# Lcressot/fhe-string-bounty

Measured on AMD Instinct MI355X. Metric: PBS/sec (whole node), higher is better.
Workload: dtype f64

## Files before the change

fhe-string-bounty_amd/csrc/engine.h:

```cpp
#pragma once
#include <hip/hip_runtime.h>
#include <stdint.h>

#include <algorithm>
#include <map>
#include <memory>
#include <mutex>
#include <string>
#include <vector>

#include "../../include/fhestr.h"
#include "blind_rotate.h"
#include "device_buffer.h"
#include "engine_settings.h"
#include "grid_spans.h"

#define FHESTR_KERNEL_REVISION "r04.2"

namespace fhe {

inline uint32_t n_ggsw(const fhe_params_t& p) {
    return p.grouping_factor > 1 ? p.n / p.grouping_factor * (1u << p.grouping_factor) : p.n;
}
inline uint64_t multi_bit_key_bit(const uint64_t* group_bits, uint32_t g, uint32_t sel) {
    uint64_t prod = 1;
    for (uint32_t b = 0; b < g; b++) prod *= group_bits[b] ^ (((sel >> (g - 1 - b)) & 1) ^ 1);
    return prod;
}

void aes128_round_keys(const uint8_t key[16], uint8_t rk[11][16]);
const uint8_t* aes_sbox();

extern thread_local std::string g_last_error;
inline int under(const char* who, hipError_t e) { return e == hipSuccess ? 0 : fail(std::string(who) + ": " + hipGetErrorString(e)); }
inline int under(const char* who, int rc) { return rc ? fail(std::string(who) + ": " + g_last_error) : 0; }

uint64_t fill_accumulator(const fhe_params_t& p, const uint64_t* table, std::vector<uint64_t>& acc);
void fill_accumulator_torus(const fhe_params_t& p, const uint64_t* box_values, std::vector<uint64_t>& acc);

struct ByteRange { const char* lo; const char* hi; };
inline bool overlap(const ByteRange& a, const ByteRange& b) { return a.lo < b.hi && b.lo < a.hi; }

struct PipeLane {
    hipStream_t stream = nullptr;
    hipEvent_t done = nullptr;
    DeviceBuffer<uint64_t> small;
    DeviceBuffer<int8_t> digits;
    std::vector<ByteRange> ins, outs;
    bool blocks(const ByteRange& in, const ByteRange& out) const {
        for (const auto& w : outs)
            if (overlap(in, w) || overlap(out, w)) return true;
        for (const auto& r : ins)
            if (overlap(out, r)) return true;
        return false;
    }
    void remember(const ByteRange& in, const ByteRange& out) { add(ins, in); add(outs, out); }
    static void add(std::vector<ByteRange>& rs, const ByteRange& a) {
        for (auto& r : rs)
            if (r.lo == a.lo && r.hi == a.hi) return;
        if (rs.size() < 32) { rs.push_back(a); return; }
        rs[0].lo = std::min(rs[0].lo, a.lo);
        rs[0].hi = std::max(rs[0].hi, a.hi);
    }
};

struct Pipeline {
    static constexpr int MAX_LANES = 4;
    PipeLane lane[MAX_LANES];
    int ready = 0;
    int width = 2;
    uint64_t calls = 0;
    hipEvent_t input_ready = nullptr;
    hipEvent_t ks_done[2] = {nullptr, nullptr}, rot_done[2] = {nullptr, nullptr};
    ByteRange prev_out[2] = {{nullptr, nullptr}, {nullptr, nullptr}};
    hipEvent_t run_start = nullptr;

    template <class F> void each_event(F f) {
        for (auto& l : lane) f(l.done);
        for (int s = 0; s < 2; s++) { f(ks_done[s]); f(rot_done[s]); }
        f(run_start);
    }
    int ensure(int n);
    hipStream_t stream_of(int q, hipStream_t engine) const { return q ? lane[q].stream : engine; }
    int wait_others();
    int wait_all(hipStream_t engine);
    void end_run();
    void destroy(int keep = 0);
    ~Pipeline() { destroy(); }
};
static_assert(EngineSettings::OVERLAP_MAX == Pipeline::MAX_LANES, "every width the settings accept has its lane");

struct Engine;
struct Packing {
    Engine* e = nullptr;
    DeviceBuffer<int8_t> key;
    fhe_packing_params_t pp{0, 0};
    DeviceBuffer<int8_t> digits;
    DeviceBuffer<uint64_t> pack_in, pack_out;
    uint32_t pack_last[5] = {0, 0, 0, 0, 0};
    DeviceBuffer<uint64_t> unpack_in, unpack_out;
    uint32_t unpack_last[4] = {0, 0, 0, 0};
    DeviceBuffer<uint64_t> narrow_in, narrow_out;
    uint32_t narrow_last[5] = {0, 0, 0, 0, 0};
    void pack_info(uint32_t out[5]) const { std::copy(pack_last, pack_last + 5, out); }
    void unpack_info(uint32_t out[4]) const { std::copy(unpack_last, unpack_last + 4, out); }
    void narrow_info(uint32_t out[5]) const { std::copy(narrow_last, narrow_last + 5, out); }

    int load_key(const fhe_packing_params_t& pp, const uint64_t* pksk);
    int pack_dev(const uint64_t* d_cts, uint32_t count, uint64_t* d_glwes);
    int pack_host(const uint64_t* cts, uint32_t count, uint64_t* glwes);
    int extract_dev(const char* who, uint32_t k, uint32_t N, const uint64_t* d_glwes, uint32_t first, uint32_t count, uint64_t* d_cts, uint32_t* chunks = nullptr);
    int unpack_dev(const uint64_t* d_glwes, uint32_t first, uint32_t count, int refresh, uint64_t* d_cts);
    int unpack_host(const uint64_t* glwes, uint32_t first, uint32_t count, int refresh, uint64_t* cts);
    int narrow_dev(const uint64_t* d_glwes, uint32_t held, uint32_t bits, uint64_t* d_narrow);
    int narrow_host(const uint64_t* glwes, uint32_t held, uint32_t bits, uint64_t* narrow);
    int widen_dev(const uint64_t* d_narrow, uint32_t held, uint32_t bits, uint64_t* d_glwes);
    int widen_shape_dev(const char* who, uint32_t k, uint32_t N, const uint64_t* d_narrow, uint32_t held, uint32_t bits, uint64_t* d_glwes);
    int unpack_narrow_dev(const uint64_t* d_narrow, uint32_t held, uint32_t bits, uint32_t first, uint32_t count, int refresh, uint64_t* d_cts);
    int unpack_narrow_host(const uint64_t* narrow, uint32_t held, uint32_t bits, uint32_t first, uint32_t count, int refresh, uint64_t* cts);

    DeviceBuffer<uint32_t> ring_key;
    fhe_packing_params_t ring_pp{0, 0};
    DeviceBuffer<uint32_t> ring_tw;
    uint32_t ring_n_inv = 0;
    DeviceBuffer<uint64_t> ring_slots;
    DeviceBuffer<unsigned char> ring_tmp;
    uint64_t ring_last[5] = {0, 0, 0, 0, 0};
    int load_ring_key(const fhe_packing_params_t& pp, const uint64_t* key);
    int ring_pack_dev(const uint64_t* d_cts, uint32_t count, uint64_t* d_glwes);
    int ring_pack_host(const uint64_t* cts, uint32_t count, uint64_t* glwes);
    int ring_ntt_host(uint32_t N, int inverse, uint32_t* polys, uint32_t count);
};

struct Transcipher {
    Engine* e = nullptr;
    uint32_t cipher = 0, max_streams = 0, bits = 0;
    uint32_t n_streams = 0;
    int32_t round = 0;
    DeviceBuffer<uint64_t> key;
    DeviceBuffer<uint64_t> ring;
    DeviceBuffer<uint64_t> pbs_in;
    DeviceBuffer<uint32_t> tables;
    DeviceBuffer<uint8_t> ivs, data;
    DeviceBuffer<uint64_t> out;
    uint32_t lut_of[20] = {};
    uint32_t warm_rounds = 0, data_rounds = 0;
    uint64_t pbs_rows = 0;
    bool timed = false;
    double phase_ms[3] = {0, 0, 0};
    uint32_t timed_rounds = 0;
    hipEvent_t ev[4] = {nullptr, nullptr, nullptr, nullptr};

    static int create(Engine& e, uint32_t cipher, const uint64_t* key_cts, uint32_t max_streams, Transcipher** out);
    ~Transcipher();
    int begin(const uint8_t* ivs_host, uint32_t streams);
    int next(const uint8_t* data_host, uint32_t n_bytes, int refresh, uint64_t* out_host, uint64_t* d_out);
    int run_round(uint32_t rows, uint32_t n_bytes, uint32_t m, uint64_t* d_blocks);
    void info(uint32_t out[8]) const;
};

struct CastKey {
    Engine* e = nullptr;
    fhe_cast_params_t cp{};
    int32_t shift = 0;
    uint32_t in_dim = 0, out_size = 0;
    DeviceBuffer<int8_t> key;
    DeviceBuffer<int8_t> digits;
    DeviceBuffer<uint64_t> rows;
    DeviceBuffer<uint64_t> bodies;
    DeviceBuffer<uint64_t> lwes;
    DeviceBuffer<uint64_t> glwes;
    DeviceBuffer<uint32_t> idx;
    DeviceBuffer<unsigned char> meta;
    DeviceBuffer<uint64_t> in, out;
    bool fused = true;
    uint32_t group = 1;
    uint32_t meta_count = 0;
    uint32_t lut = 0;
    bool lut_ready = false;
    uint32_t last = 0;
    double v_in = 1.0;

    static int create(Engine& e, const fhe_cast_params_t& cp, const uint64_t* key, CastKey** out);
    int set_group(uint32_t group);
    int gate(const char* who) const;
    int keyswitch_dev(const uint64_t* d_src, uint32_t first, uint32_t count, bool packed, uint64_t* d_rows);
    int cast_dev(const uint64_t* d_src, uint32_t first, uint32_t count, bool packed, int mode, uint64_t* d_out);
    int cast_host(const uint64_t* src, uint32_t first, uint32_t count, bool packed, int mode, uint64_t* out);
    int cast_narrow_dev(const uint64_t* d_narrow, uint32_t held, uint32_t bits, uint32_t first, uint32_t count, int mode, uint64_t* d_out);
    int cast_narrow_host(const uint64_t* narrow, uint32_t held, uint32_t bits, uint32_t first, uint32_t count, int mode, uint64_t* out);
    int digits_host(const uint64_t* src, uint32_t first, uint32_t count, bool packed, int8_t* out, size_t* bytes);
    void info(uint32_t out[8]) const;
};

struct Engine {
    std::recursive_mutex mu;
    fhe_params_t p{};
    int device = 0;
    hipStream_t stream = nullptr;
    hipStream_t own_stream = nullptr;
    std::map<std::vector<uint64_t>, uint32_t> lut_dedup;
    std::vector<hipEvent_t> ring;
    size_t ring_used = 0;
    const BrVariant* variant = nullptr;
    const BrVariant* variant_large = nullptr;
    int cu_count = 256;
    uint32_t max_grid[3] = {0x7FFFFFFFu, 65535u, 65535u};
    GridSpans spans(uint64_t count, int axis) const { return grid_spans(count, max_grid[axis]); }
    int one_span(const char* who, uint64_t count, int axis) const {
        if (spans(count, axis).spans == 1) return 0;
        return fail(std::string(who) + ": grid." + "xyz"[axis] + " = " + std::to_string(count) + " does not fit one launch (the device allows " +
                    std::to_string(max_grid[axis]) + ")");
    }
    EngineSettings cfg;
    int pipeline = 0;
    Pipeline pipe;
    int sync_all_streams() { return pipe.wait_all(stream); }
    int leave_pipelined_run() {
        if (!pipeline) return 0;
        if (sync_all_streams()) return 1;
        pipe.end_run();
        return 0;
    }
    template <class T>
    int reserve_idle(DeviceBuffer<T>& b, size_t need) {
        if (b.bytes >= need) return 0;
        if (b.ptr && sync_all_streams()) return 1;
        return b.reserve(need);
    }
    int shadow_fit = -1;

    DeviceBuffer<uint32_t> d_ksk_packed;
    DeviceBuffer<uint64_t> d_ksk_rowsum;
    DeviceBuffer<int8_t> d_ksk_mfma;
    DeviceBuffer<double> d_fbsk;
    DeviceBuffer<double> d_fbsk_dense;
    DeviceBuffer<uint64_t> d_luts;
    uint32_t n_luts = 0;

    DeviceBuffer<uint64_t> d_in, d_out, d_pool;
    DeviceBuffer<uint32_t> d_idx;
    DeviceBuffer<unsigned char> d_meta;
    DeviceBuffer<uint64_t> d_compact;
    DeviceBuffer<unsigned char> d_ws;
    DeviceBuffer<uint32_t> d_slot_exp;
    MultiCuRuntime multi_cu;
    uint32_t ks_last[5] = {0, 0, 0, 0, 0};
    Packing packing;
    DeviceBuffer<uint32_t> refresh_idx;
    std::vector<std::unique_ptr<Transcipher>> transciphers;
    std::vector<std::unique_ptr<CastKey>> cast_keys;

    static int create(const fhe_params_t& p, int device, Engine** out);
    ~Engine();
    int use();
    int set_variant(int logR);
    int allow_rotate_lds();
    int load_keys(const uint64_t* bsk_std, const uint64_t* ksk);
    int load_seeded_keys(const uint8_t ksk_seed[16], const uint64_t* ksk_bodies, const uint8_t bsk_seed[16], const uint64_t* bsk_bodies,
                         uint64_t* bsk_std_out, uint64_t* ksk_out);
    int expand_seeded_lwe(const uint8_t* seeds, const uint64_t* bodies, uint32_t count, uint64_t* d_out, uint64_t* host_out);
    int expand_compact_list(const uint64_t* list, uint32_t count, uint64_t* d_out, uint64_t* host_out);
    int expand_compact_list_dev(const uint64_t* d_list, uint32_t count, uint64_t* d_out);
    int generate_keys(const uint64_t* glwe_sk, const uint64_t* small_sk, const uint8_t seed[32],
                      uint64_t* bsk_std_out, uint64_t* ksk_out);
    int install_keys(DeviceBuffer<uint64_t>&& d_ksk_std, DeviceBuffer<uint64_t>&& d_bsk_std);
    int convert_polys(const uint64_t* d_std, double* d_out, uint32_t n_polys);
    int convert_dense_key(const uint64_t* d_std, uint32_t n_polys);
    int probe_slot_exponents();
    uint64_t fill_accumulator(const uint64_t* table, std::vector<uint64_t>& acc) const { return fhe::fill_accumulator(p, table, acc); }
    int lut_upload_dedup(const std::vector<uint64_t>& acc, uint32_t* id);
    int set_stream(hipStream_t s, bool use_own);
    int lut_upload(const uint64_t* acc, uint32_t* id);
    int lut_download(uint32_t id, uint64_t* acc);
    int ensure_batch(uint32_t count);
    int timing_events(hipEvent_t*& e4);
    int check_lut_idx(const uint32_t* lut_idx, uint32_t count) const;

    int launch_keyswitch(const uint64_t* d_big, uint64_t* d_sm, uint32_t count, DeviceBuffer<int8_t>& digits, hipStream_t on = nullptr, bool shadow = false);
    int launch_blind_rotate(const uint64_t* d_sm, const uint32_t* d_lut_idx, uint64_t* d_big, uint32_t count, hipStream_t on = nullptr, bool two_per_cu = false,
                            bool one_workgroup_only = false);
    bool shadow_keyswitch_fits();
    int refresh_rows_dev(uint64_t* d_cts, uint32_t count);
    uint32_t rotate_registers() const;
    void keyswitch_info(uint32_t info[6]) const;
    int ks_pbs_dev(const uint64_t* d_big_in, const uint32_t* d_lut_idx, uint64_t* d_big_out, uint32_t count, bool allow_pipeline = false);
    int ks_pbs_host(const uint64_t* in, const uint32_t* lut_idx, uint64_t* out, uint32_t count);
    int keyswitch_host(const uint64_t* in, uint64_t* out_small, uint32_t count);
    int pbs_host(const uint64_t* in_small, const uint32_t* lut_idx, uint64_t* out, uint32_t count);
    int pbs_ks_host(const uint64_t* in_small, const uint32_t* lut_idx, uint64_t* out_small, uint32_t count);
    int lincomb_dev(const uint64_t* d_pool, const uint32_t* d_off, const uint32_t* d_src,
                    const int32_t* d_coeff, const uint64_t* d_cst, uint64_t* d_out, uint32_t jobs);
    int lincomb_rows_dev(const uint64_t* d_pool, const uint32_t* d_off, const uint32_t* d_src, const int32_t* d_coeff, const uint64_t* d_cst,
                         uint64_t* d_out, uint32_t jobs, uint32_t row_words);
    int lincomb_batch_dev(const uint64_t* d_pool, const uint32_t* d_off, const uint32_t* d_src, const int32_t* d_coeff,
                          const uint64_t* d_cst, uint64_t* d_out, uint32_t jobs, uint32_t instances, uint32_t src_slot, uint32_t src_inst,
                          uint32_t out_job, uint32_t out_inst, const uint32_t* d_lut_in, uint32_t* d_lut_out);
    int restride_dev(const uint64_t* d_in, uint64_t* d_out, uint32_t slots, uint32_t instances, uint32_t in_slot, uint32_t in_inst,
                     uint32_t out_slot, uint32_t out_inst);
    int lincomb_host(const uint64_t* pool, uint32_t pool_count, const uint32_t* off, const uint32_t* src,
                     const int32_t* coeff, const uint64_t* cst, uint64_t* out, uint32_t jobs);
    int transcipher_init_host(uint32_t cipher, uint32_t S, const uint64_t* key, const uint8_t* ivs, uint64_t* ring);
    int transcipher_gather_host(uint32_t cipher, uint32_t S, int32_t round, uint32_t rows, const uint64_t* ring, const uint64_t* key, const uint8_t* ivs,
                                const uint8_t* data, uint32_t n_bytes, uint32_t m, uint64_t* pbs_in, uint32_t* tables);
    int transcipher_apply_host(uint32_t cipher, uint32_t S, int32_t round, const uint64_t* ring, uint32_t n_bytes, uint32_t m, uint64_t* out);
    int last_kernel_ms(float ms[2]);
    int kernel_times(double total_ms[2], uint32_t* calls, bool reset);
    int synchronize();
};

struct Seed256;
size_t compact_dim(const fhe_params_t& p);
int compact_pk_generate(const fhe_params_t& p, const uint64_t* big_sk, const Seed256& seed, uint64_t* pk, int threads);

int params_supported(const fhe_params_t& p);
int packing_params_check(const fhe_params_t& p, const fhe_packing_params_t& pp);
void packing_unpack_noise(const fhe_params_t& p, const fhe_packing_params_t& pp, double out[2]);
void narrow_noise(const fhe_params_t& p, const fhe_packing_params_t& pp, uint32_t bits, double out[3]);

}

struct fhe_plan;
struct fhe_engine {
    fhe::Engine* impl;
    std::vector<std::pair<std::string, fhe_plan*>> str_plans;
};
```

fhe-string-bounty_amd/csrc/pbs_kernels.hip.h:

```cpp
#pragma once
#include <type_traits>
#include "negacyclic_fft.hip.h"

namespace fhe {

#ifdef FHESTR_WALL
__device__ unsigned long long g_wall[4096 * 2];
#endif
#ifdef FHESTR_STAMPS
constexpr int STAMP_SEGS = 10;
__device__ unsigned long long g_stamps[4096 * 8 * STAMP_SEGS];
#define FHE_STAMP_DECL unsigned long long stamp_acc[STAMP_SEGS] = {}; unsigned long long stamp_prev = 0
#define FHE_STAMP(idx)                                                                                   \
    do {                                                                                                 \
        __builtin_amdgcn_sched_barrier(0);                                                               \
        unsigned long long _t;                                                                           \
        asm volatile("s_memtime %0\n\ts_waitcnt lgkmcnt(0)" : "=s"(_t)::"memory");                       \
        __builtin_amdgcn_sched_barrier(0);                                                               \
        if ((idx) >= 0) stamp_acc[(idx) < 0 ? 0 : (idx)] += _t - stamp_prev;                             \
        stamp_prev = _t;                                                                                 \
    } while (0)
#else
#define FHE_STAMP_DECL do {} while (0)
#define FHE_STAMP(idx) do {} while (0)
#endif

__device__ uint32_t g_cu_tickets[2048];

struct BlindRotateArgs {
    const uint64_t* lwe_small;
    const uint32_t* lut_idx;
    const uint64_t* luts;
    const double* fbsk;
    uint64_t* lwe_out;
    uint32_t n;
    uint32_t base_log;
    uint32_t batch;
    uint32_t grouping;
    uint32_t fair_shift;
};

__device__ __forceinline__ uint32_t decomp_init_state(uint64_t x, uint32_t bL) {
    uint32_t t = (uint32_t)(x >> (63 - bL));
    return ((t + 1u) >> 1) & ((1u << bL) - 1u);
}
__device__ __forceinline__ int32_t decomp_next_digit(uint32_t& state, uint32_t base_log) {
    const uint32_t mask = (1u << base_log) - 1u;
    uint32_t res = state & mask;
    state >>= base_log;
    uint32_t carry = ((res - 1u) | state) & res;
    carry >>= base_log - 1;
    state += carry;
    return (int32_t)(res - (carry << base_log));
}
__device__ __forceinline__ uint64_t decomp_init_state64(uint64_t x, uint32_t bL) {
    const uint64_t t = x >> (63 - bL);
    return ((t + 1ull) >> 1) & ((1ull << bL) - 1ull);
}
__device__ __forceinline__ int32_t decomp_next_digit64(uint64_t& state, uint32_t base_log) {
    const uint64_t mask = (1ull << base_log) - 1ull;
    uint64_t res = state & mask;
    state >>= base_log;
    uint64_t carry = ((res - 1ull) | state) & res;
    carry >>= base_log - 1;
    state += carry;
    return (int32_t)(uint32_t)(res - (carry << base_log));
}
__device__ __forceinline__ int32_t decomp_single_digit(uint64_t x, uint32_t b) {
    const uint32_t t = (uint32_t)(x >> 32) >> (31 - b);
    const uint32_t res = __builtin_amdgcn_ubfe(t + 1u, 1u, b);
    const uint32_t half = 1u << (b - 1);
    return (int32_t)(res - ((res + (half - 1u)) & (half << 1)));
}
__device__ __forceinline__ uint32_t decomp_bias_constant(uint32_t b) {
    uint32_t c = 0x80000000u - (1u << (31 - b));
    asm volatile("" : "+s"(c));
    return c;
}
__device__ __forceinline__ uint32_t decomp_single_biased(uint64_t x, uint32_t b, uint32_t bias_constant) {
    const uint32_t hi = (uint32_t)(x >> 32);
    return __builtin_amdgcn_ubfe(hi + bias_constant, 32u - b, b);
}
__device__ __forceinline__ cplx digit_point(uint32_t lo_biased, uint32_t hi_biased, cplx tw, cplx kb) {
    const double a = (double)lo_biased, b = (double)hi_biased;
    cplx r;
    r.re = fma(a, tw.re, fma(-b, tw.im, kb.re));
    r.im = fma(a, tw.im, fma(b, tw.re, kb.im));
    return r;
}
__device__ __forceinline__ uint32_t modulus_switch(uint64_t x, int logN) {
    uint64_t o = x >> (64 - logN - 2);
    return (uint32_t)((o + 1) >> 1);
}

template <int LOGN>
__device__ __forceinline__ void modswitch_mask(const uint64_t* lwe, uint32_t steps, uint32_t* lds_d, uint32_t threads, bool extprod) {
    for (uint32_t i = threadIdx.x; i < steps; i += threads) {
        const uint64_t a = lwe[i];
        lds_d[i] = extprod ? 0u : (a == 0 ? 0xFFFFFFFFu : modulus_switch(a, LOGN));
    }
}
template <class PL, int N>
__device__ __forceinline__ void twist_consts(int tau, uint32_t base_log_total, cplx* twist, cplx* twbias) {
#pragma unroll
    for (int m = 0; m < PL::R; m++) {
        double sn, cs;
        sincospi((double)PL::point(tau, m) / (double)N, &sn, &cs);
        twist[m].re = cs; twist[m].im = sn;
        const double cb = -(double)((1u << (base_log_total - 1)) - 1u);
        twbias[m].re = cb * (cs - sn);
        twbias[m].im = cb * (cs + sn);
    }
}
template <int LOGN>
__device__ __forceinline__ uint64_t rotated_lut_coeff(const uint64_t* lut_poly, uint32_t j, uint32_t d_body) {
    constexpr uint32_t N = 1u << LOGN;
    const uint32_t rem = d_body & (N - 1);
    const bool odd = (d_body >> LOGN) & 1;
    const bool neg = ((j + rem) >= N) != odd;
    const uint64_t v = lut_poly[(j + rem) & (N - 1)];
    return neg ? (0 - v) : v;
}
template <int N, int K1>
__device__ __forceinline__ void extract_store(uint64_t* out, uint32_t p, uint32_t j, uint64_t v) {
    if (p == (uint32_t)(K1 - 1)) {
        if (j == 0) out[(size_t)(K1 - 1) * N] = v;
    } else {
        if (j == 0) out[(size_t)p * N] = v;
        else out[(size_t)p * N + (N - j)] = 0 - v;
    }
}
template <int N>
__device__ __forceinline__ cplx torus_point_to_fourier_input(uint64_t a, uint64_t b, int j) {
    cplx z;
    z.re = i64_to_f64(a) * (5.421010862427522e-20 / (N / 2));
    z.im = i64_to_f64(b) * (5.421010862427522e-20 / (N / 2));
    double sn, cs;
    sincospi((double)j / (double)N, &sn, &cs);
    cplx w; w.re = cs; w.im = sn;
    return cmul(z, w);
}

typedef unsigned int u32x4_t __attribute__((ext_vector_type(4)));
__device__ __forceinline__ auto key_resource(const double* fbsk, size_t bytes) {
    return __builtin_amdgcn_make_buffer_rsrc(const_cast<double*>(fbsk), 0, bytes < 0x7FFFFFF0u ? (int)bytes : 0x7FFFFFF0, 0x00020000);
}
template <class RSRC>
__device__ __forceinline__ double2 key_load(RSRC rsrc, uint32_t voff, uint32_t soff) {
    const u32x4_t v = __builtin_amdgcn_raw_buffer_load_b128(rsrc, (int)voff, (int)soff, 0);
    double2 d;
    __builtin_memcpy(&d, &v, 16);
    return d;
}

template <class PL>
__device__ __forceinline__ uint32_t acc_slot_of(uint32_t j) { return (uint32_t)PL::acc_slot((int)j); }

template <class PL>
__host__ __device__ constexpr int swap_wave_bits() {
    if constexpr (PL::SWAP) return PL::LOGW; else return 0;
}
template <class PL, int LOGN>
struct Rotation {
    int32_t oddmask;
    uint32_t rem;
    int32_t qb8;
    uint32_t rbits8;
    __device__ __forceinline__ Rotation(uint32_t d, int tau) {
        rem = d & ((1u << LOGN) - 1);
        oddmask = -(int32_t)((d >> LOGN) & 1);
        if constexpr (PL::SWAP) {
            constexpr int LW = swap_wave_bits<PL>();
            const int w = __builtin_amdgcn_readfirstlane(tau >> 6), lane = tau & 63;
            const int rr = (int)(rem & ((1u << LW) - 1));
            qb8 = (int32_t)((uint32_t)((lane - (int)(rem >> LW) - (w < rr ? 1 : 0)) << 3) + ((uint32_t)oddmask & 0x80000000u));
            rbits8 = (uint32_t)((w - rr) & ((1 << LW) - 1)) << (LOGN - LW + 3);
        } else {
            qb8 = 0; rbits8 = 0;
        }
    }
    __device__ __forceinline__ void source(int tau, int m, int h, uint32_t& slot, uint32_t& neg) const {
        static_assert(!PL::SWAP, "swap plan: use source_bytes");
        const uint32_t j = (uint32_t)PL::point(tau, m) + (uint32_t)h * PL::P;
        neg = (uint32_t)(((int32_t)(j - rem) >> 31) ^ oddmask);
        slot = acc_slot_of<PL>((j - rem) & ((1u << LOGN) - 1));
    }
    __device__ __forceinline__ void source_bytes(int m, int h, uint32_t row_base, uint32_t& address, uint32_t& neg) const {
        constexpr int LW = swap_wave_bits<PL>();
        const int32_t q8 = qb8 + ((PL::point(0, m) + h * PL::P) >> LW) * 8;
        neg = (uint32_t)(q8 >> 31);
        address = ((uint32_t)q8 & (((1u << (LOGN - LW)) - 1) << 3)) | row_base;
    }
    __device__ __forceinline__ void source_bytes_q8(int m, int h, uint32_t row_base, uint32_t& address, int32_t& q8) const {
        constexpr int LW = swap_wave_bits<PL>();
        q8 = qb8 + ((PL::point(0, m) + h * PL::P) >> LW) * 8;
        address = ((uint32_t)q8 & (((1u << (LOGN - LW)) - 1) << 3)) | row_base;
    }
};

__device__ __forceinline__ uint32_t biased_difference(uint64_t gathered, int32_t q8, uint64_t own_nk, uint32_t b) {
    const uint32_t sm = (uint32_t)(q8 >> 31), nsm = ~sm;
    const uint64_t s = gathered + (own_nk ^ (((uint64_t)nsm << 32) | nsm));
    return __builtin_amdgcn_ubfe((uint32_t)(s >> 32) ^ sm, 32u - b, b);
}

typedef __attribute__((address_space(3))) const uint64_t lds_cu64_t;
__device__ __forceinline__ uint32_t lds_address(const void* p) {
    return (uint32_t)(uintptr_t)(__attribute__((address_space(3))) const void*)p;
}
__device__ __forceinline__ uint64_t lds_load_u64(uint32_t byte_address) { return *(lds_cu64_t*)(uintptr_t)byte_address; }

template <int LOGN, int LOGR, int K1, int L>
struct BrCfg {
    static constexpr int N = 1 << LOGN;
    static constexpr int P = N / 2;
    using PL = typename PlanFor<LOGN - 1, LOGR>::type;
    static constexpr int R = PL::R;
    static constexpr int T = PL::T;
    static constexpr int THREADS = K1 * T;
    static constexpr int PLANE = P + 2;
    static constexpr int GROUP_SLOTS = 2 * P + 4;
    static constexpr size_t LDS_FIXED = (size_t)K1 * N * 8  + (size_t)K1 * GROUP_SLOTS * 8  +
                                        (size_t)K1 * GROUP_SLOTS * 8 ;
    static size_t lds_bytes(uint32_t n) { return LDS_FIXED + (size_t)n * 4; }
};

template <int LOGN, int LOGR, int K1, int L>
__global__ void __launch_bounds__((BrCfg<LOGN, LOGR, K1, L>::THREADS))
bsk_convert_kernel(const uint64_t* __restrict__ bsk_std, double* __restrict__ fbsk, uint32_t n_polys) {
    using CFG = BrCfg<LOGN, LOGR, K1, L>;
    using PL = typename CFG::PL;
    constexpr int N = CFG::N, P = CFG::P, R = CFG::R, T = CFG::T;
    extern __shared__ __align__(16) unsigned char smem[];
    const int g = threadIdx.x / T, tau = threadIdx.x % T;
    double* xre = reinterpret_cast<double*>(smem) + (size_t)g * CFG::GROUP_SLOTS;
    double* xim = xre + CFG::PLANE;
    const uint32_t poly = blockIdx.x * K1 + g;
    const bool active = poly < n_polys;
    FftConsts<PL> fc;
    fft_init_consts<PL>(fc, tau);
    cplx x[R];
#pragma unroll
    for (int m = 0; m < R; m++) {
        const int j = PL::point(tau, m);
        uint64_t a = active ? bsk_std[(size_t)poly * N + j] : 0;
        uint64_t b = active ? bsk_std[(size_t)poly * N + j + P] : 0;
        x[m] = torus_point_to_fourier_input<N>(a, b, j);
    }
    fft_forward<PL>(x, fc, xre, xim, tau);
    if (active) {
        double2* out = reinterpret_cast<double2*>(fbsk) + (size_t)poly * P;
#pragma unroll
        for (int rho = 0; rho < R; rho++) out[rho * T + tau] = make_double2(x[rho].re, x[rho].im);
    }
}

template <int LOGN, int LOGR, int K1, int L, bool EXTPROD = false>
__global__ void __launch_bounds__((BrCfg<LOGN, LOGR, K1, L>::THREADS))
blind_rotate_kernel(BlindRotateArgs args) {
    using CFG = BrCfg<LOGN, LOGR, K1, L>;
    static_assert(!EXTPROD || !CFG::PL::SWAP, "N = 2048 has its own multi-bit kernels");
    using PL = typename CFG::PL;
    constexpr int N = CFG::N, P = CFG::P, R = CFG::R, T = CFG::T;
    extern __shared__ __align__(16) unsigned char smem[];
    uint64_t* lds_acc = reinterpret_cast<uint64_t*>(smem);
    double* lds_x = reinterpret_cast<double*>(smem + (size_t)K1 * N * 8);
    double* lds_f = lds_x + (size_t)K1 * CFG::GROUP_SLOTS;
    uint32_t* lds_d = reinterpret_cast<uint32_t*>(lds_f + (size_t)K1 * CFG::GROUP_SLOTS);

    int g = threadIdx.x / T;
    const int tau = threadIdx.x % T;
    if constexpr (T % 64 == 0) g = __builtin_amdgcn_readfirstlane(g);
#ifdef FHESTR_WALL
    const unsigned long long wall_t0 = __builtin_amdgcn_s_memrealtime();
#endif
    const uint32_t sample = blockIdx.x < args.batch ? blockIdx.x : blockIdx.x % args.batch;
    const uint32_t n = args.n;
    const uint64_t* lwe = args.lwe_small + (size_t)sample * (n + 1);
    const uint64_t* lut = args.luts + (size_t)(args.lut_idx ? args.lut_idx[sample] : 0) * K1 * N;
    uint64_t* my_acc = lds_acc + (size_t)g * N;
    const uint32_t my_acc_address = lds_address(my_acc);
    if (PL::SWAP && (my_acc_address & (8u * N - 1u))) __builtin_trap();
    double* xre = lds_x + (size_t)g * CFG::GROUP_SLOTS;
    double* xim = xre + CFG::PLANE;
    const uint32_t bL = args.base_log * L;
    const uint32_t dbias = decomp_bias_constant(bL <= 31 ? bL : 31);

    const uint32_t steps = EXTPROD ? n / args.grouping : n;
    modswitch_mask<LOGN>(lwe, steps, lds_d, CFG::THREADS, EXTPROD);

    FftConsts<PL> fc;
    fft_init_consts<PL>(fc, tau);
    cplx twist[R], twbias[R];
#pragma unroll
    for (int m = 0; m < R; m++) {
        double sn, cs;
        sincospi((double)PL::point(tau, m) / (double)N, &sn, &cs);
        twist[m].re = cs; twist[m].im = sn;
        const double cb = -(double)((1u << (args.base_log * L - 1)) - 1u);
        twbias[m].re = cb * (cs - sn);
        twbias[m].im = cb * (cs + sn);
    }

    uint64_t acc_lo[R], acc_hi[R];
    {
        const uint32_t d = modulus_switch(lwe[n], LOGN);
        const uint32_t rem = d & (N - 1);
        const bool odd = (d >> LOGN) & 1;
#pragma unroll
        for (int m = 0; m < R; m++) {
#pragma unroll
            for (int h = 0; h < 2; h++) {
                const uint32_t j = PL::point(tau, m) + h * P;
                const uint32_t src = (j + rem) & (N - 1);
                const bool neg = ((j + rem) >= (uint32_t)N) != odd;
                uint64_t v = lut[(size_t)g * N + src];
                v = neg ? (0 - v) : v;
                if (h == 0) acc_lo[m] = v; else acc_hi[m] = v;
            }
        }
    }
#pragma unroll
    for (int m = 0; m < R; m++) {
        my_acc[acc_slot_of<PL>(PL::point(tau, m))] = acc_lo[m];
        my_acc[acc_slot_of<PL>(PL::point(tau, m) + P)] = acc_hi[m];
    }
    __syncthreads();

    const double2* fbsk = reinterpret_cast<const double2*>(args.fbsk);
    constexpr size_t GGSW_ELEMS = (size_t)L * K1 * K1 * P;

    uint32_t d_next = lds_d[0];
    const uint32_t key_off = (uint32_t)tau * 16u;
    if constexpr (EXTPROD) fbsk += (size_t)sample * steps * GGSW_ELEMS;
    const auto key_rsrc = key_resource(reinterpret_cast<const double*>(fbsk), (size_t)steps * GGSW_ELEMS * 16);
    FHE_STAMP_DECL;
    FHE_STAMP(-1);
    for (uint32_t i = 0; i < steps; i++) {
        const uint32_t d = (uint32_t)__builtin_amdgcn_readfirstlane((int)d_next);
        d_next = lds_d[i + 1 < steps ? i + 1 : i];
        if (d == 0xFFFFFFFFu) continue;
        const Rotation<PL, LOGN> rot(d, tau);

        const double2* bk0 = fbsk + (size_t)i * GGSW_ELEMS;
        double2 bpre[K1][R];
        {
#pragma unroll
            for (int r = 0; r < K1; r++) {
                const int row = (g + r) % K1;
#pragma unroll
                for (int rho = 0; rho < R; rho++) {
                    const uint32_t soff = (uint32_t)((i * GGSW_ELEMS + (size_t)(L - 1) * K1 * K1 * P +
                                                      ((size_t)row * K1 + g) * P + rho * T) * 16);
                    bpre[r][rho] = key_load(key_rsrc, key_off, soff);
                }
            }
        }

        uint32_t st_lo[R], st_hi[R];
        uint32_t row_base = my_acc_address | rot.rbits8;
        if constexpr (PL::SWAP) asm volatile("" : "+s"(row_base));
#pragma unroll
        for (int m = 0; m < R; m++) {
#pragma unroll
            for (int h = 0; h < 2; h++) {
                if constexpr (EXTPROD) {
                    const uint64_t own = h == 0 ? acc_lo[m] : acc_hi[m];
                    const uint32_t st = L == 1 ? decomp_single_biased(own, bL, dbias) : decomp_init_state(own, bL);
                    if (h == 0) st_lo[m] = st; else st_hi[m] = st;
                    continue;
                }
                uint32_t sm32;
                uint64_t gathered;
                if constexpr (PL::SWAP) {
                    uint32_t address;
                    rot.source_bytes(m, h, row_base, address, sm32);
                    gathered = lds_load_u64(address);
                } else {
                    uint32_t slot;
                    rot.source(tau, m, h, slot, sm32);
                    gathered = my_acc[slot];
                }
                const uint64_t sm = ((uint64_t)sm32 << 32) | sm32;
                const uint64_t v = (gathered ^ sm) - sm;
                const uint64_t own = h == 0 ? acc_lo[m] : acc_hi[m];
                const uint32_t st = L == 1 ? decomp_single_biased(v - own, bL, dbias) : decomp_init_state(v - own, bL);
                if (h == 0) st_lo[m] = st; else st_hi[m] = st;
            }
        }

        FHE_STAMP(0);
        cplx outf[R];
        if constexpr (PL::SWAP) {
            static_assert(!PL::SWAP || L == 1, "swap plan: single decomposition level only");
            cplx x[K1][R];
#pragma unroll
            for (int m = 0; m < R; m++) x[0][m] = digit_point(st_lo[m], st_hi[m], twist[m], twbias[m]);
#ifdef FHESTR_WALL
    if (threadIdx.x == 0 && blockIdx.x < 4096) {
        uint32_t xcc;
        asm volatile("s_getreg_b32 %0, hwreg(HW_REG_XCC_ID)" : "=s"(xcc));
        g_wall[blockIdx.x * 2] = __builtin_amdgcn_s_memrealtime() - wall_t0;
        g_wall[blockIdx.x * 2 + 1] = xcc & 7u;
    }
#endif
#ifdef FHESTR_STAMPS
            swap10_fwd_stage1(x[0], fc, xre, xim, tau);
            FHE_STAMP(1);
            wave_local_fence();
            swap10_fwd_stage2(x[0], fc, xre, xim, tau);
            FHE_STAMP(2);
            wave_local_fence();
            swap10_fwd_stage3(x[0], fc, xre, xim, tau);
            FHE_STAMP(3);
#else
            swap10_forward_head(x[0], fc, xre, xim, tau);
#endif
            __syncthreads();
            FHE_STAMP(4);
#pragma unroll
            for (int r = 0; r < K1; r++) {
                const int row = (g + r) % K1;
                const double* rre = lds_x + (size_t)row * CFG::GROUP_SLOTS;
                swap10_forward_tail(x[r], rre, rre + CFG::PLANE, tau);
            }
#pragma unroll
            for (int r = 0; r < K1; r++) {
#pragma unroll
                for (int rho = 0; rho < R; rho++) {
                    const double2 bv = bpre[r][rho];
                    const cplx f = x[r][rho];
                    if (r == 0) {
                        outf[rho].re = bv.x * f.re - bv.y * f.im;
                        outf[rho].im = bv.x * f.im + bv.y * f.re;
                    } else {
                        outf[rho].re = fma(bv.x, f.re, fma(-bv.y, f.im, outf[rho].re));
                        outf[rho].im = fma(bv.x, f.im, fma(bv.y, f.re, outf[rho].im));
                    }
                }
            }
            double* fre = lds_f + (size_t)g * CFG::GROUP_SLOTS;
            double* fim = fre + CFG::PLANE;
            FHE_STAMP(5);
            swap10_inverse_head(outf, fre, fim, tau);
            FHE_STAMP(6);
            __syncthreads();
            FHE_STAMP(7);
            swap10_inverse_tail(outf, fc, fre, fim, tau);
            FHE_STAMP(8);
        } else {
#pragma unroll
        for (int it = 0; it < L; it++) {
            const int lvl_idx = L - 1 - it;
            cplx x[R];
#pragma unroll
            for (int m = 0; m < R; m++) {
                if (L == 1) { x[m] = digit_point(st_lo[m], st_hi[m], twist[m], twbias[m]); continue; }
                cplx z;
                z.re = (double)decomp_next_digit(st_lo[m], args.base_log);
                z.im = (double)decomp_next_digit(st_hi[m], args.base_log);
                x[m] = cmul(z, twist[m]);
            }
            fft_forward<PL>(x, fc, xre, xim, tau);
            if (it > 0) __syncthreads();
            {
                double* fre = lds_f + (size_t)g * CFG::GROUP_SLOTS;
                double* fim = fre + CFG::PLANE;
#pragma unroll
                for (int rho = 0; rho < R; rho++) {
                    fre[rho * T + tau] = x[rho].re;
                    fim[rho * T + tau] = x[rho].im;
                }
            }
            __syncthreads();
            const double2* bk = bk0 + (size_t)lvl_idx * K1 * K1 * P;
#pragma unroll
            for (int r = 0; r < K1; r++) {
                const int row = (g + r) % K1;
                const double* fre = lds_f + (size_t)row * CFG::GROUP_SLOTS;
                const double* fim = fre + CFG::PLANE;
#pragma unroll
                for (int rho = 0; rho < R; rho++) {
                    const double2 bv = it == 0 ? bpre[r][rho] : bk[((size_t)row * K1 + g) * P + rho * T + tau];
                    cplx f;
                    if (r == 0) {
                        f = x[rho];
                    } else {
                        f.re = fre[rho * T + tau];
                        f.im = fim[rho * T + tau];
                    }
                    if (it == 0 && r == 0) {
                        outf[rho].re = bv.x * f.re - bv.y * f.im;
                        outf[rho].im = bv.x * f.im + bv.y * f.re;
                    } else {
                        outf[rho].re = fma(bv.x, f.re, fma(-bv.y, f.im, outf[rho].re));
                        outf[rho].im = fma(bv.x, f.im, fma(bv.y, f.re, outf[rho].im));
                    }
                }
            }
        }

        fft_inverse<PL>(outf, fc, xre, xim, tau);
        }
#pragma unroll
        for (int m = 0; m < R; m++) {
            cplx t = cmul_conj(outf[m], twist[m]);
            if constexpr (EXTPROD) {
                acc_lo[m] = from_torus(t.re);
                acc_hi[m] = from_torus(t.im);
                continue;
            }
            acc_lo[m] += from_torus(t.re);
            acc_hi[m] += from_torus(t.im);
            my_acc[acc_slot_of<PL>(PL::point(tau, m))] = acc_lo[m];
            my_acc[acc_slot_of<PL>(PL::point(tau, m) + P)] = acc_hi[m];
            FHE_PIN_ORDER();
        }
        __syncthreads();
        FHE_STAMP(9);
    }
#ifdef FHESTR_STAMPS
    if ((threadIdx.x & 63) == 0 && blockIdx.x < 4096)
        for (int sg = 0; sg < STAMP_SEGS; sg++)
            g_stamps[((size_t)blockIdx.x * 8 + (threadIdx.x >> 6)) * STAMP_SEGS + sg] = stamp_acc[sg];
#endif

    if (blockIdx.x >= args.batch) return;
    uint64_t* out = args.lwe_out + (size_t)sample * ((size_t)(K1 - 1) * N + 1);
#pragma unroll
    for (int m = 0; m < R; m++) {
#pragma unroll
        for (int h = 0; h < 2; h++) {
            const uint32_t j = PL::point(tau, m) + h * P;
            const uint64_t v = h == 0 ? acc_lo[m] : acc_hi[m];
            if (g == K1 - 1) {
                if (j == 0) out[(size_t)(K1 - 1) * N] = v;
            } else {
                if (j == 0) out[(size_t)g * N] = v;
                else out[(size_t)g * N + (N - j)] = 0 - v;
            }
        }
    }
}

template <int LOGN, int LOGR, int K1, int L, bool KEYPF = false>
struct BrWideCfg {
    static constexpr int N = 1 << LOGN;
    static constexpr int P = N / 2;
    static constexpr bool OWN_PLAN = LOGN == 12 && LOGR == 2;
    static constexpr bool LDS_TWIDDLES = OWN_PLAN;
    using PL = typename std::conditional<OWN_PLAN, FftSwap11, typename PlanFor<LOGN - 1, LOGR>::type>::type;
    static constexpr int R = PL::R;
    static constexpr int T = PL::T;
    static constexpr int THREADS = T;
    static constexpr int PLANE = P + 2;
    static constexpr int GROUP_SLOTS = 2 * P + 4;
    static constexpr bool TW_IN_LDS = !PL::SWAP && PL::NTW > 4;
    static constexpr size_t LDS_TW = TW_IN_LDS ? (size_t)FftHybridConsts<PL>::ENTRIES * 16
                                     : LDS_TWIDDLES ? (size_t)FftSwapLdsConsts<PL>::ENTRIES * 16 : 0;
    static constexpr size_t LDS_FIXED = (size_t)K1 * N * 8  + (size_t)K1 * GROUP_SLOTS * 8  + LDS_TW;
    static constexpr bool ACC_IN_LDS = LOGN >= 12;
    static constexpr bool PREFETCH_ALL = K1 * K1 * R * 4 <= 64 || KEYPF;
};

template <int LOGN, int LOGR, int K1, int L, bool KEYPF = false>
__global__ void __launch_bounds__((BrWideCfg<LOGN, LOGR, K1, L, KEYPF>::THREADS))
blind_rotate_wide_kernel(BlindRotateArgs args) {
    using CFG = BrWideCfg<LOGN, LOGR, K1, L, KEYPF>;
    using PL = typename CFG::PL;
    constexpr int N = CFG::N, P = CFG::P, R = CFG::R, T = CFG::T;
    extern __shared__ __align__(16) unsigned char smem[];
    uint64_t* lds_acc = reinterpret_cast<uint64_t*>(smem);
    double* lds_x = reinterpret_cast<double*>(smem + (size_t)K1 * N * 8);
    double2* lds_tw = reinterpret_cast<double2*>(lds_x + (size_t)K1 * CFG::GROUP_SLOTS);
    uint32_t* lds_d = reinterpret_cast<uint32_t*>(lds_tw + CFG::LDS_TW / 16);

    const int tau = threadIdx.x;
#ifdef FHESTR_WALL
    const unsigned long long wall_t0 = __builtin_amdgcn_s_memrealtime();
#endif
    const uint32_t sample = blockIdx.x;
    const uint32_t n = args.n;
    const uint64_t* lwe = args.lwe_small + (size_t)sample * (n + 1);
    const uint64_t* lut = args.luts + (size_t)(args.lut_idx ? args.lut_idx[sample] : 0) * K1 * N;
    const uint32_t acc_address = lds_address(lds_acc);
    if (PL::SWAP && (acc_address & (8u * N - 1u))) __builtin_trap();
    const uint32_t bL = args.base_log * L;
    const uint32_t dbias = decomp_bias_constant(bL <= 31 ? bL : 31);
    if (args.fair_shift && threadIdx.x == 0) {
        uint32_t fair_parity;
        uint32_t hw, xcc;
        asm volatile("s_getreg_b32 %0, hwreg(HW_REG_HW_ID)" : "=s"(hw));
        asm volatile("s_getreg_b32 %0, hwreg(HW_REG_XCC_ID)" : "=s"(xcc));
        fair_parity = atomicAdd(&g_cu_tickets[((xcc & 7u) << 8) | ((hw >> 8) & 0xFFu)], 1u) & 1u;
        reinterpret_cast<uint32_t*>(lds_x)[0] = fair_parity;
    }

    for (uint32_t i = threadIdx.x; i < n; i += CFG::THREADS) {
        const uint64_t a = lwe[i];
        lds_d[i] = a == 0 ? 0xFFFFFFFFu : modulus_switch(a, LOGN);
    }

    typename std::conditional<CFG::LDS_TWIDDLES, FftSwapLdsConsts<PL>,
                              typename std::conditional<CFG::TW_IN_LDS, FftHybridConsts<PL>, FftConsts<PL>>::type>::type fc;
    if constexpr (CFG::LDS_TWIDDLES) {
        FftSwapLdsConsts<PL>::fill(lds_tw, threadIdx.x, CFG::THREADS);
        fc.init(lds_tw, tau);
    } else if constexpr (CFG::TW_IN_LDS) {
        FftHybridConsts<PL>::fill(lds_tw, threadIdx.x, CFG::THREADS);
        fc.init(lds_tw, tau);
    } else {
        fft_init_consts<PL>(fc, tau);
    }
    cplx twist[R], twbias[R];
    twist_consts<PL, N>(tau, args.base_log * L, twist, twbias);

    constexpr bool ACC_LDS = CFG::ACC_IN_LDS;
    uint64_t acc_lo[ACC_LDS ? 1 : K1][R], acc_hi[ACC_LDS ? 1 : K1][R];
    auto own_slot = [&](int p, int m, int h) { return (size_t)p * N + acc_slot_of<PL>(PL::point(tau, m) + h * P); };
    {
        const uint32_t d = modulus_switch(lwe[n], LOGN);
#pragma unroll
        for (int p = 0; p < K1; p++)
#pragma unroll
            for (int m = 0; m < R; m++)
#pragma unroll
                for (int h = 0; h < 2; h++) {
                    const uint32_t j = PL::point(tau, m) + h * P;
                    const uint64_t v = rotated_lut_coeff<LOGN>(lut + (size_t)p * N, j, d);
                    if constexpr (!ACC_LDS) { if (h == 0) acc_lo[p][m] = v; else acc_hi[p][m] = v; }
                    lds_acc[(size_t)p * N + acc_slot_of<PL>(j)] = v;
                }
    }
    __syncthreads();

    const double2* fbsk = reinterpret_cast<const double2*>(args.fbsk);
    constexpr size_t GGSW_ELEMS = (size_t)L * K1 * K1 * P;
    const uint32_t key_off = (uint32_t)tau * 16u;
    const auto key_rsrc = key_resource(args.fbsk, (size_t)n * GGSW_ELEMS * 16);

    const uint32_t fair_shift = args.fair_shift;
    uint32_t fair_turn = 0;
    if (fair_shift) {
        fair_turn = (uint32_t)__builtin_amdgcn_readfirstlane((int)reinterpret_cast<uint32_t*>(lds_x)[0]);
        __syncthreads();
    }
    uint32_t d_next = lds_d[0];
    for (uint32_t i = 0; i < n; i++) {
        const uint32_t d = (uint32_t)__builtin_amdgcn_readfirstlane((int)d_next);
        d_next = lds_d[i + 1 < n ? i + 1 : i];
        if (d == 0xFFFFFFFFu) continue;
        if (fair_shift) {
            if ((((uint32_t)(__builtin_amdgcn_s_memrealtime() >> fair_shift)) ^ fair_turn) & 1u) __builtin_amdgcn_s_setprio(1);
            else __builtin_amdgcn_s_setprio(0);
        }
        const Rotation<PL, LOGN> rot(d, tau);
        const double2* bk0 = fbsk + (size_t)i * GGSW_ELEMS;

        double2 bpre[CFG::PREFETCH_ALL ? K1 : 1][CFG::PREFETCH_ALL ? K1 : 1][R];
        if (CFG::PREFETCH_ALL) {
#pragma unroll
            for (int row = 0; row < K1; row++)
#pragma unroll
                for (int col = 0; col < K1; col++)
#pragma unroll
                    for (int rho = 0; rho < R; rho++)
                        bpre[row][col][rho] = key_load(key_rsrc, key_off,
                            (uint32_t)((i * GGSW_ELEMS + (size_t)(L - 1) * K1 * K1 * P + ((size_t)row * K1 + col) * P + rho * T) * 16));
        }

        uint32_t st_lo[K1][R], st_hi[K1][R];
        const uint64_t nk = ~((uint64_t)dbias << 32);
        uint32_t row_base[K1];
#pragma unroll
        for (int p = 0; p < K1; p++) {
            row_base[p] = (acc_address + (uint32_t)p * 8u * N) | rot.rbits8;
            if constexpr (PL::SWAP) asm volatile("" : "+s"(row_base[p]));
        }
        constexpr bool GATHER_BATCH = PL::SWAP && L == 1 && !ACC_LDS;
        if constexpr (GATHER_BATCH) {
            uint64_t gv[K1][R][2];
            int32_t q8v[R][2];
#pragma unroll
            for (int m = 0; m < R; m++)
#pragma unroll
                for (int h = 0; h < 2; h++) {
                    uint32_t address;
                    rot.source_bytes_q8(m, h, row_base[0], address, q8v[m][h]);
#pragma unroll
                    for (int p = 0; p < K1; p++) gv[p][m][h] = lds_load_u64(address + (uint32_t)p * 8u * N);
                }
            FHE_PIN_ORDER();
#pragma unroll
            for (int p = 0; p < K1; p++)
#pragma unroll
                for (int m = 0; m < R; m++) {
                    st_lo[p][m] = biased_difference(gv[p][m][0], q8v[m][0], acc_lo[p][m] + nk, bL);
                    st_hi[p][m] = biased_difference(gv[p][m][1], q8v[m][1], acc_hi[p][m] + nk, bL);
                }
        }
#pragma unroll
        for (int p = 0; p < (GATHER_BATCH ? 0 : K1); p++)
#pragma unroll
            for (int m = 0; m < R; m++)
#pragma unroll
                for (int h = 0; h < 2; h++) {
                    uint32_t sm32;
                    uint64_t gathered;
                    if constexpr (PL::SWAP) {
                        uint32_t address;
                        rot.source_bytes(m, h, row_base[p], address, sm32);
                        gathered = lds_load_u64(address);
                    } else {
                        uint32_t slot;
                        rot.source(tau, m, h, slot, sm32);
                        gathered = lds_acc[(size_t)p * N + slot];
                    }
                    const uint64_t sm = ((uint64_t)sm32 << 32) | sm32;
                    const uint64_t v = (gathered ^ sm) - sm;
                    uint64_t own;
                    if constexpr (ACC_LDS) own = lds_acc[own_slot(p, m, h)];
                    else own = h == 0 ? acc_lo[p][m] : acc_hi[p][m];
                    const uint32_t st = L == 1 ? decomp_single_biased(v - own, bL, dbias) : decomp_init_state(v - own, bL);
                    if (h == 0) st_lo[p][m] = st; else st_hi[p][m] = st;
                }

        cplx outf[K1][R];
#pragma unroll
        for (int it = 0; it < L; it++) {
            const int lvl_idx = L - 1 - it;
            cplx x[K1][R];
#pragma unroll
            for (int p = 0; p < K1; p++)
#pragma unroll
                for (int m = 0; m < R; m++) {
                    if (L == 1) {
                        if constexpr (CFG::LDS_TWIDDLES) {
                            const int32_t cbi = (int32_t)((1u << (args.base_log * L - 1)) - 1u);
                            cplx z;
                            z.re = (double)((int32_t)st_lo[p][m] - cbi);
                            z.im = (double)((int32_t)st_hi[p][m] - cbi);
                            x[p][m] = cmul(z, twist[m]);
                        } else {
                            x[p][m] = digit_point(st_lo[p][m], st_hi[p][m], twist[m], twbias[m]);
                        }
                        continue;
                    }
                    cplx z;
                    z.re = (double)decomp_next_digit(st_lo[p][m], args.base_log);
                    z.im = (double)decomp_next_digit(st_hi[p][m], args.base_log);
                    x[p][m] = cmul(z, twist[m]);
                }
            fft_forward_multi<PL, K1>(x, fc, lds_x, CFG::GROUP_SLOTS, CFG::PLANE, tau);
            const double2* bk = bk0 + (size_t)lvl_idx * K1 * K1 * P;
#pragma unroll
            for (int row = 0; row < K1; row++) {
#pragma unroll
                for (int col = 0; col < K1; col++)
#pragma unroll
                    for (int rho = 0; rho < R; rho++) {
                        const double2 bv = (CFG::PREFETCH_ALL && it == 0)
                                               ? bpre[CFG::PREFETCH_ALL ? row : 0][CFG::PREFETCH_ALL ? col : 0][rho]
                                               : bk[((size_t)row * K1 + col) * P + rho * T + tau];
                        const cplx f = x[row][rho];
                        if (it == 0 && row == 0) {
                            outf[col][rho].re = bv.x * f.re - bv.y * f.im;
                            outf[col][rho].im = bv.x * f.im + bv.y * f.re;
                        } else {
                            outf[col][rho].re = fma(bv.x, f.re, fma(-bv.y, f.im, outf[col][rho].re));
                            outf[col][rho].im = fma(bv.x, f.im, fma(bv.y, f.re, outf[col][rho].im));
                        }
                    }
            }
            if (it + 1 < L) __syncthreads();
        }

        fft_inverse_multi<PL, K1>(outf, fc, lds_x, CFG::GROUP_SLOTS, CFG::PLANE, tau);
#pragma unroll
        for (int p = 0; p < K1; p++)
#pragma unroll
            for (int m = 0; m < R; m++) {
                cplx t = cmul_conj(outf[p][m], twist[m]);
                if constexpr (ACC_LDS) {
                    lds_acc[own_slot(p, m, 0)] += from_torus(t.re);
                    lds_acc[own_slot(p, m, 1)] += from_torus(t.im);
                } else {
                acc_lo[p][m] += from_torus(t.re);
                acc_hi[p][m] += from_torus(t.im);
                lds_acc[(size_t)p * N + acc_slot_of<PL>(PL::point(tau, m))] = acc_lo[p][m];
                lds_acc[(size_t)p * N + acc_slot_of<PL>(PL::point(tau, m) + P)] = acc_hi[p][m];
                }
                FHE_PIN_ORDER();
            }
        __syncthreads();
    }

#ifdef FHESTR_WALL
    if (threadIdx.x == 0 && blockIdx.x < 4096) {
        g_wall[blockIdx.x * 2] = __builtin_amdgcn_s_memrealtime() - wall_t0;
        g_wall[blockIdx.x * 2 + 1] = wall_t0;
    }
#endif
    uint64_t* out = args.lwe_out + (size_t)sample * ((size_t)(K1 - 1) * N + 1);
#pragma unroll
    for (int p = 0; p < K1; p++)
#pragma unroll
        for (int m = 0; m < R; m++)
#pragma unroll
            for (int h = 0; h < 2; h++) {
                uint64_t v;
                if constexpr (ACC_LDS) v = lds_acc[own_slot(p, m, h)];
                else v = h == 0 ? acc_lo[p][m] : acc_hi[p][m];
                extract_store<N, K1>(out, p, PL::point(tau, m) + h * P, v);
            }
}

template <int LOGN, int LOGR, int K1, int L>
__global__ void __launch_bounds__((BrWideCfg<LOGN, LOGR, K1, L>::THREADS))
bsk_convert_wide_kernel(const uint64_t* __restrict__ bsk_std, double* __restrict__ fbsk, uint32_t n_polys) {
    using CFG = BrWideCfg<LOGN, LOGR, K1, L>;
    using PL = typename CFG::PL;
    constexpr int N = CFG::N, P = CFG::P, R = CFG::R, T = CFG::T;
    extern __shared__ __align__(16) unsigned char smem[];
    double* planes = reinterpret_cast<double*>(smem);
    const int tau = threadIdx.x;
    const uint32_t poly = blockIdx.x;
    if (poly >= n_polys) return;
    FftConsts<PL> fc;
    fft_init_consts<PL>(fc, tau);
    cplx x[R];
#pragma unroll
    for (int m = 0; m < R; m++) {
        const int j = PL::point(tau, m);
        x[m] = torus_point_to_fourier_input<N>(bsk_std[(size_t)poly * N + j], bsk_std[(size_t)poly * N + j + P], j);
    }
    fft_forward<PL>(x, fc, planes, planes + CFG::PLANE, tau);
    double2* out = reinterpret_cast<double2*>(fbsk) + (size_t)poly * P;
#pragma unroll
    for (int rho = 0; rho < R; rho++) out[rho * T + tau] = make_double2(x[rho].re, x[rho].im);
}

}
```

Before: 131,600.

## Restructure blind-rotate step head for N=2048 single-level wide kernel

```diff
diff --git a/fhe-string-bounty_amd/csrc/engine.h b/fhe-string-bounty_amd/csrc/engine.h
--- a/fhe-string-bounty_amd/csrc/engine.h
+++ b/fhe-string-bounty_amd/csrc/engine.h
@@ -15,7 +15,7 @@
 #include "engine_settings.h"
 #include "grid_spans.h"
 
-#define FHESTR_KERNEL_REVISION "r04.2"
+#define FHESTR_KERNEL_REVISION "r04.3"
 
 namespace fhe {
 
diff --git a/fhe-string-bounty_amd/csrc/pbs_kernels.hip.h b/fhe-string-bounty_amd/csrc/pbs_kernels.hip.h
--- a/fhe-string-bounty_amd/csrc/pbs_kernels.hip.h
+++ b/fhe-string-bounty_amd/csrc/pbs_kernels.hip.h
@@ -166,12 +166,13 @@
     uint32_t rem;
     int32_t qb8;
     uint32_t rbits8;
-    __device__ __forceinline__ Rotation(uint32_t d, int tau) {
+    __device__ __forceinline__ Rotation(uint32_t d, int tau) : Rotation(d, tau, __builtin_amdgcn_readfirstlane(tau >> 6)) {}
+    __device__ __forceinline__ Rotation(uint32_t d, int tau, int w) {
         rem = d & ((1u << LOGN) - 1);
         oddmask = -(int32_t)((d >> LOGN) & 1);
         if constexpr (PL::SWAP) {
             constexpr int LW = swap_wave_bits<PL>();
-            const int w = __builtin_amdgcn_readfirstlane(tau >> 6), lane = tau & 63;
+            const int lane = tau & 63;
             const int rr = (int)(rem & ((1u << LW) - 1));
             qb8 = (int32_t)((uint32_t)((lane - (int)(rem >> LW) - (w < rr ? 1 : 0)) << 3) + ((uint32_t)oddmask & 0x80000000u));
             rbits8 = (uint32_t)((w - rr) & ((1 << LW) - 1)) << (LOGN - LW + 3);
@@ -209,6 +210,8 @@
     return (uint32_t)(uintptr_t)(__attribute__((address_space(3))) const void*)p;
 }
 __device__ __forceinline__ uint64_t lds_load_u64(uint32_t byte_address) { return *(lds_cu64_t*)(uintptr_t)byte_address; }
+typedef __attribute__((address_space(3))) const uint32_t lds_cu32_t;
+__device__ __forceinline__ uint32_t lds_load_u32(uint32_t byte_address) { return *(lds_cu32_t*)(uintptr_t)byte_address; }
 
 template <int LOGN, int LOGR, int K1, int L>
 struct BrCfg {
@@ -561,6 +564,7 @@
     static constexpr size_t LDS_FIXED = (size_t)K1 * N * 8  + (size_t)K1 * GROUP_SLOTS * 8  + LDS_TW;
     static constexpr bool ACC_IN_LDS = LOGN >= 12;
     static constexpr bool PREFETCH_ALL = K1 * K1 * R * 4 <= 64 || KEYPF;
+    static constexpr bool STEP_HEAD = LOGN == 11 && LOGR == 2 && L == 1;
 };
 
 template <int LOGN, int LOGR, int K1, int L, bool KEYPF = false>
@@ -645,28 +649,48 @@
         fair_turn = (uint32_t)__builtin_amdgcn_readfirstlane((int)reinterpret_cast<uint32_t*>(lds_x)[0]);
         __syncthreads();
     }
-    uint32_t d_next = lds_d[0];
+    constexpr bool STEP_HEAD = CFG::STEP_HEAD;
+    constexpr bool GATHER_BATCH = PL::SWAP && L == 1 && !ACC_LDS;
+    static_assert(!STEP_HEAD || (GATHER_BATCH && CFG::PREFETCH_ALL), "the reordered head is the batched gather's, with the whole key prefetched");
+    const int wave = __builtin_amdgcn_readfirstlane(tau >> 6);
+    const uint32_t mask_last = lds_address(lds_d) + 4u * (n - 1), mask_lane = lds_address(lds_d) + 4u * ((uint32_t)tau & 63u);
+    auto mask_window = [&](uint32_t i0) { return lds_load_u32(min(mask_lane + 4u * i0, mask_last)); };
+    uint32_t d_window = STEP_HEAD ? mask_window(0) : 0;
+    uint32_t d_next = STEP_HEAD ? 0 : lds_d[0];
+    unsigned long long slice_clock = 0;
+    if constexpr (STEP_HEAD) slice_clock = __builtin_amdgcn_s_memrealtime();
+    FHE_STAMP_DECL;
+    FHE_STAMP(-1);
     for (uint32_t i = 0; i < n; i++) {
-        const uint32_t d = (uint32_t)__builtin_amdgcn_readfirstlane((int)d_next);
-        d_next = lds_d[i + 1 < n ? i + 1 : i];
+        uint32_t d;
+        if constexpr (STEP_HEAD) {
+            d = (uint32_t)__builtin_amdgcn_readlane((int)d_window, (int)(i & 63u));
+            if ((i & 63u) == 63u) d_window = mask_window(i + 1);
+        } else {
+            d = (uint32_t)__builtin_amdgcn_readfirstlane((int)d_next);
+            d_next = lds_d[i + 1 < n ? i + 1 : i];
+        }
         if (d == 0xFFFFFFFFu) continue;
         if (fair_shift) {
-            if ((((uint32_t)(__builtin_amdgcn_s_memrealtime() >> fair_shift)) ^ fair_turn) & 1u) __builtin_amdgcn_s_setprio(1);
+            if constexpr (!STEP_HEAD) slice_clock = __builtin_amdgcn_s_memrealtime();
+            if ((((uint32_t)(slice_clock >> fair_shift)) ^ fair_turn) & 1u) __builtin_amdgcn_s_setprio(1);
             else __builtin_amdgcn_s_setprio(0);
         }
-        const Rotation<PL, LOGN> rot(d, tau);
+        const Rotation<PL, LOGN> rot(d, tau, wave);
         const double2* bk0 = fbsk + (size_t)i * GGSW_ELEMS;
 
         double2 bpre[CFG::PREFETCH_ALL ? K1 : 1][CFG::PREFETCH_ALL ? K1 : 1][R];
-        if (CFG::PREFETCH_ALL) {
+        auto prefetch_key = [&](int row, int col, int rho) {
+            bpre[row][col][rho] = key_load(key_rsrc, key_off,
+                (uint32_t)((i * GGSW_ELEMS + (size_t)(L - 1) * K1 * K1 * P + ((size_t)row * K1 + col) * P + rho * T) * 16));
+        };
+        if constexpr (CFG::PREFETCH_ALL && !STEP_HEAD) {
 #pragma unroll
             for (int row = 0; row < K1; row++)
 #pragma unroll
                 for (int col = 0; col < K1; col++)
 #pragma unroll
-                    for (int rho = 0; rho < R; rho++)
-                        bpre[row][col][rho] = key_load(key_rsrc, key_off,
-                            (uint32_t)((i * GGSW_ELEMS + (size_t)(L - 1) * K1 * K1 * P + ((size_t)row * K1 + col) * P + rho * T) * 16));
+                    for (int rho = 0; rho < R; rho++) prefetch_key(row, col, rho);
         }
 
         uint32_t st_lo[K1][R], st_hi[K1][R];
@@ -677,7 +701,7 @@
             row_base[p] = (acc_address + (uint32_t)p * 8u * N) | rot.rbits8;
             if constexpr (PL::SWAP) asm volatile("" : "+s"(row_base[p]));
         }
-        constexpr bool GATHER_BATCH = PL::SWAP && L == 1 && !ACC_LDS;
+        FHE_STAMP(0);
         if constexpr (GATHER_BATCH) {
             uint64_t gv[K1][R][2];
             int32_t q8v[R][2];
@@ -697,6 +721,15 @@
                 for (int m = 0; m < R; m++) {
                     st_lo[p][m] = biased_difference(gv[p][m][0], q8v[m][0], acc_lo[p][m] + nk, bL);
                     st_hi[p][m] = biased_difference(gv[p][m][1], q8v[m][1], acc_hi[p][m] + nk, bL);
+                    if constexpr (STEP_HEAD) {
+                        FHE_PIN_ORDER();
+#pragma unroll
+                        for (int e = 0; e < K1; e++) {
+                            const int idx = (p * R + m) * K1 + e;
+                            prefetch_key(idx / (K1 * R), idx / R % K1, idx % R);
+                        }
+                        FHE_PIN_ORDER();
+                    }
                 }
         }
 #pragma unroll
@@ -724,6 +757,7 @@
                     const uint32_t st = L == 1 ? decomp_single_biased(v - own, bL, dbias) : decomp_init_state(v - own, bL);
                     if (h == 0) st_lo[p][m] = st; else st_hi[p][m] = st;
                 }
+        FHE_STAMP(1);
 
         cplx outf[K1][R];
 #pragma unroll
@@ -791,9 +825,28 @@
                 lds_acc[(size_t)p * N + acc_slot_of<PL>(PL::point(tau, m) + P)] = acc_hi[p][m];
                 }
                 FHE_PIN_ORDER();
+                if constexpr (STEP_HEAD) {
+                    if (p == K1 - 1 && m == 0) {
+                        slice_clock = __builtin_amdgcn_s_memrealtime();
+                        FHE_PIN_ORDER();
+                    }
+                }
             }
         __syncthreads();
-    }
+        FHE_STAMP(2);
+    }
+#ifdef FHESTR_STAMPS
+    {
+        FHE_STAMP(-1);
+        unsigned long long rt;
+        asm volatile("s_memrealtime %0\n\ts_waitcnt lgkmcnt(0)" : "=s"(rt)::"memory");
+        FHE_STAMP(3);
+        FHE_STAMP(4);
+        if ((threadIdx.x & 63) == 0 && blockIdx.x < 4096)
+            for (int sg = 0; sg < STAMP_SEGS; sg++)
+                g_stamps[((size_t)blockIdx.x * 8 + (threadIdx.x >> 6)) * STAMP_SEGS + sg] = stamp_acc[sg];
+    }
+#endif
 
 #ifdef FHESTR_WALL
     if (threadIdx.x == 0 && blockIdx.x < 4096) {
```

Result: faster. 134,400, median of 4 (+2.1%).
